# althonos/pyrodigal

Hardware: AMD Instinct MI355X
Metric: Mbp/sec gene-called (meta mode) (higher is better)
Workload: dtype f64; 1 GPU; 100000x20kbp_gc30-70_meta; contigs=100000, bases=2000000000, models=16, contigs_rank0=100000, sub_batch_contigs=6250, contexts_per_gpu=4, genes_all_ranks=2908995, steps_issued=a join of the contexts and a gather per step

## Files before the change

### pyrodigal_amd/csrc/pipeline.hip

```cpp

#include "pga_internal.h"
#include "pipeline.h"
#include <atomic>
#include "dev_common.h"
#include "dpw_core.h"

namespace {

enum { NA = 0, NG = 1, NC = 2, NT = 3, NN = 6 };

__device__ __forceinline__ int find_contig(const ContigDesc* __restrict__ ct, int n, int64_t g) {
    int lo = 0, hi = n - 1;
    while (lo < hi) { int mid = (lo + hi + 1) >> 1; if (ct[mid].base <= g) lo = mid; else hi = mid - 1; }
    return lo;
}

__device__ __forceinline__ int block_contig(const ContigDesc* __restrict__ ct, int n, int64_t block_first, int64_t g, int* s_slot) {
    int c = block_search_le([&](const int k) { return ct[k].base; }, n, block_first, s_slot);
    while (c + 1 < n && ct[c + 1].base <= g) c++;
    return c;
}
__device__ __forceinline__ int block_chain(const ChainDesc* __restrict__ ch, int n, int64_t block_first, int64_t g, int* s_slot) {
    int c = block_search_le([&](const int k) { return ch[k].off; }, n, block_first, s_slot);
    while (c + 1 < n && ch[c + 1].off <= g) c++;
// ... 2184 lines not shown
        if (tid < 256) SM.mot.mk0[tid >> 6][tid & 63] = tm->mot_wt[0][tid >> 6][tid & 63];
#pragma unroll
        for (int e = tid; e < 1024; e += TILE) SM.mot.mk1[e >> 8][e & 255] = tm->mot_wt[1][e >> 8][e & 255];
    }
    if (tid < nj) {
        const SsMmChain C = mm[T.j0 + tid];
        s_item0[tid] = C.item0; s_n[tid] = C.n; s_rdelta[tid] = C.rdelta; s_lf[tid] = C.len_first; s_off[tid] = C.off; s_raw[tid] = C.raw;
    }
    __syncthreads();
    mark(0);
    const int item = T.item0 + tid;
    int lo = 0, hi = nj - 1;
    while (lo < hi) { const int mid = (lo + hi + 1) >> 1; if (s_item0[mid] <= item) lo = mid; else hi = mid - 1; }
    if (item < s_item0[lo] + s_n[lo]) {
    const ulonglong2* const rp = (const ulonglong2*)&rec[item + s_rdelta[lo]];
    const ulonglong2 ra = rp[0], rb = rp[1];
    const int64_t raw = s_raw[lo], g0 = s_off[lo];
    const uint32_t len_first = s_lf[lo];
    const unsigned long long ucodes = ra.x, w1 = ra.y, w2 = rb.x, w3 = rb.y;
    const int i = (int)(unsigned)w3;
    const double cs_raw = ca.cscore_raw[raw + i];
    const int64_t g = g0 + i;
    const int L = (int)(len_first & 0x7fffffffu);
    const bool first = (len_first >> 31) != 0;
    const unsigned long long zm = w1 & ((1ull << 42) - 1ull);
    const int nups = (int)((w1 >> 42) & 63u), start = (int)((w1 >> 48) & 63u), type = (int)((w1 >> 54) & 3u);
    const int strand = ((w1 >> 56) & 1u) ? -1 : 1;
    const bool e0 = (w1 >> 57) & 1u, conv = (w1 >> 58) & 1u, ups_near_edge = (w1 >> 59) & 1u, ups_first = (w1 >> 60) & 1u, ups_later = (w1 >> 61) & 1u;
    const unsigned isA = (unsigned)(w2 & 0xfffffu) << 1, isG = (unsigned)((w2 >> 20) & 0xfffffu) << 1;
    const int stop3 = (int)(w2 >> 40);
    const long orf = (long)(w3 >> 32);
    const bool is_meta = sp.is_meta != 0;
    const double st_wt = SM.st_wt;
    const bool stop_missing = !codon_is_stop(stop3 & 0xff, (stop3 >> 8) & 0xff, (stop3 >> 16) & 0xff, SM.tt);
    const bool edge_in = e0 || (conv && !first);
    mark(1);
    int rbs0 = 0, rbs1 = 0, m_ndx = 0, m_len = 0, m_sp = 0, m_si = 0;
    double m_score = 0.0;
    const bool search_sd = !edge_in && SM.uses_sd, search_mot = !edge_in && !SM.uses_sd;
    auto midx = [&](const int k, const int t2) { return (int)((zm >> (2 * (21 - (18 + k - t2)))) & ((1ull << (2 * (k + 3))) - 1ull)); };
    auto msi = [](const int t2) { return t2 <= 2 ? 3 : (t2 <= 4 ? 2 : (t2 >= 11 ? 1 : 0)); };
    auto upstream = [&]() {
        double v = 0.0;
        unsigned lo32 = (unsigned)ucodes, hi32 = (unsigned)(ucodes >> 32);
        if (nups == 32) {
#pragma unroll
            for (int q = 0; q < 16; q++) { v += SM.ups[q][(lo32 >> (2 * q)) & 3u]; if ((q & 7) == 7) __builtin_amdgcn_sched_barrier(0); }
#pragma unroll
            for (int q = 0; q < 16; q++) { v += SM.ups[16 + q][(hi32 >> (2 * q)) & 3u]; if ((q & 7) == 7) __builtin_amdgcn_sched_barrier(0); }
        } else {
            for (int q = 0; q < nups; q++) v += SM.ups[q][(int)(ucodes >> (2 * q)) & 3];
        }
        return v;
    };
    double u = 0.0;
    if (search_sd) {
        unsigned pats[3] = {0u, 0u, 0u};
#pragma unroll
        for (int q = 0; q < 15; q++) {
            const unsigned a6 = (isA >> (15 - q)) & 63u, g6 = (isG >> (15 - q)) & 63u;
            const unsigned pat = ((a6 >> 5) & 1u) | (((g6 >> 4) & 1u) << 1) | (((g6 >> 3) & 1u) << 2) | (((a6 >> 2) & 1u) << 3) |
                                 (((g6 >> 1) & 1u) << 4) | ((g6 & 1u) << 5);
            pats[q / 5] |= pat << (6 * (q % 5));
        }
#pragma unroll
        for (int q = 0; q < 15; q++) {
            if (start - 20 + q < 0 && strand == 1) continue;
            const unsigned pat = (pats[q / 5] >> (6 * (q % 5))) & 63u;
            const unsigned he = SM.lut[(q << 6) | pat], hm = SM.lut[((15 + q) << 6) | pat];
            if (he > 1u) { const int a = sd_pick(he, SM.rbs_wt); if (a > rbs0) rbs0 = a; }
            if (hm > 1u) { const int b = sd_pick(hm, SM.rbs_wt); if (b > rbs1) rbs1 = b; }
        }
    } else if (search_mot) {
        double bsc = -100.0; int bsp = 0, bsi = 0, blen = 0, bndx = 0;
#pragma unroll 1
        for (int k = 3; k >= 0; k--) {
            const int stride = k == 0 ? 64 : (k == 1 ? 256 : 4096);
            const double* __restrict__ gt = &tm->mot_wt[k][0][0];
            const double* lt = k == 1 ? &SM.mot.mk1[0][0] : &SM.mot.mk0[0][0];
            double scv[13];
            if (k >= 2) {
#pragma unroll
                for (int t2 = 0; t2 < 13; t2++) scv[t2] = 18 + k - t2 > start ? -1000.0 : gt[msi(t2) * stride + midx(k, t2)];
            } else {
#pragma unroll
                for (int t2 = 0; t2 < 13; t2++) scv[t2] = 18 + k - t2 > start ? -1000.0 : lt[msi(t2) * stride + midx(k, t2)];
            }
#pragma unroll
            for (int t2 = 0; t2 < 13; t2++)
                if (scv[t2] > bsc) { bsc = scv[t2]; bsi = msi(t2); bsp = 15 - t2; blen = k + 3; bndx = midx(k, t2); }
        }
        if (bsc == -4.0 || bsc < SM.no_mot + 0.69) { m_score = SM.no_mot; }
        else { m_ndx = bndx; m_len = blen; m_si = bsi; m_sp = bsp & 15; m_score = bsc; }
    }
    if (!edge_in) u = upstream();
    mark(2);
    double edge_gene = 0;
    if (edge_in) edge_gene += 1;
    if (stop_missing) edge_gene += 1;

    double tscore, uscore, rscore, sscore, cscore = cs_raw;
    if (edge_in) {
        tscore = 0.74 * st_wt / edge_gene; uscore = 0.0; rscore = 0.0;
    } else {
        tscore = SM.type_wt[type] * st_wt;
        const double r1 = SM.rbs_wt[rbs0], r2 = SM.rbs_wt[rbs1];
        const double sd = fmax(r1, r2) * st_wt;
        if (SM.uses_sd) rscore = sd;
        else { rscore = st_wt * m_score; if (rscore < sd && SM.no_mot > -0.5) rscore = sd; }
        uscore = u;
        if (ups_near_edge || (first ? ups_first : ups_later)) uscore += -1.00 * st_wt;
    }
    bool edge_now = edge_in;
    if (conv && !edge_in) {
        edge_gene += 1; edge_now = true; tscore = 0.0;
        uscore = 0.74 * st_wt / edge_gene; rscore = 0.0;
    }
    if (!edge_now && edge_gene == 1) uscore -= 0.5 * 0.74 * st_wt;
    if (edge_gene == 0 && orf < 250) {
        const double negf = 250.0 / (float)orf, posf = (float)orf / 250.0;
        rscore *= rscore < 0 ? negf : posf;
        uscore *= uscore < 0 ? negf : posf;
        tscore *= tscore < 0 ? negf : posf;
    }
    if (is_meta && L < 3000 && edge_gene == 0 && (cscore < 5.0 || orf < 120))
        cscore -= 7.5 * fmax(0.0, (3000.0 - L) / 2700.0);
    sscore = tscore + rscore + uscore;
    if (cscore < 0.0) {
        if (edge_gene > 0 && !edge_now) {
            if (!is_meta || L > 1500) sscore -= st_wt; else sscore -= 10.31 - 0.004 * L;
        } else if (is_meta && L < 3000 && edge_now) {
            const double mml = sqrt((double)L) * 5.0;
            if (orf >= mml) { if (cscore >= 0) cscore = -1.0; sscore = 0.0; uscore = 0.0; }
        } else sscore -= 0.5;
    } else if (is_meta && cscore < 5.0 && orf < 120 && sscore < 0.0) sscore -= st_wt;
    mark(3);
    ca.cscore[g] = cscore; ca.sscore[g] = sscore; ca.rscore[g] = rscore; ca.uscore[g] = uscore; ca.tscore[g] = tscore;
    ca.mot_score[g] = m_score; ca.mot_ndx[g] = m_ndx;
    ca.mot_len[g] = (uint8_t)m_len; ca.mot_spacer[g] = (uint8_t)m_sp; ca.mot_spacendx[g] = (uint8_t)m_si;
    ca.rbs[2 * g] = (uint8_t)rbs0; ca.rbs[2 * g + 1] = (uint8_t)rbs1;
    ca.edge[g] = (uint8_t)edge_now;
    if (sp.cs_out != nullptr) sp.cs_out[g] = cscore + sscore;
    mark(4);
    }
}

struct OvlChain {
    const int32_t* __restrict__ ndx; const int32_t* __restrict__ stv; const uint8_t* __restrict__ typ; const int8_t* __restrict__ str;
    const double* __restrict__ cs; const double* __restrict__ ss; const double* __restrict__ rs; const double* __restrict__ us;
    int n;
    const double* __restrict__ css = nullptr;
};
constexpr int OV_SPEC = 16;
__device__ __forceinline__ unsigned overlap_neighbours(const int32_t* __restrict__ ndx, const int32_t* __restrict__ stv, const uint8_t* __restrict__ typ,
                                                       const int8_t* __restrict__ str, const int n, const int i, const int maxov) {
    const int my = ndx[i];
    const bool fwd = str[i] == 1;
    bool ended = false;
    unsigned elig = 0;
    constexpr int OV_NEAR = 10;
#pragma unroll
    for (int k = 0; k < OV_SPEC; k++) {
        if (k == OV_NEAR && ended) break;
        const int j = fwd ? i + 3 - k : i - 3 + k;
        const int jj = min(max(j, 0), n - 1);
        const int nd = ndx[jj], sv = stv[jj], ty = typ[jj], sd = str[jj];
        bool stop_here, ok;
        if (fwd) {
            stop_here = j < 0 || (j < n && nd <= my + 2 && nd + maxov < my);
            ok = j >= 0 && j < n && nd <= my + 2 && sd == 1 && ty != PGA_T_STOP && sv > my;
        } else {
            stop_here = j >= n || (j >= 0 && nd >= my - 2 && nd - maxov > my);
            ok = j >= 0 && j < n && nd >= my - 2 && sd == -1 && ty != PGA_T_STOP && sv < my;
        }
        ended = ended || stop_here;
        if (ok && !ended) {
            elig |= 1u << k;
            if (k < 15 && (fwd ? (my + 2 == nd || my == nd + 1) : (nd + 2 == my || nd == my + 1))) elig |= 0x10000u << k;
        }
    }
    return elig | (ended ? 0x80000000u : 0u);
}

__device__ __forceinline__ void overlapping_starts_of(const OvlChain& C, const int i, const ModelConst* __restrict__ mc, const int maxov,
                                                      int& sp0, int& sp1, int& sp2, const unsigned neighbours) {
    const int32_t* __restrict__ ndx = C.ndx; const int32_t* __restrict__ stv = C.stv;
    const uint8_t* __restrict__ typ = C.typ; const int8_t* __restrict__ str = C.str;
    const double* __restrict__ cs = C.cs; const double* __restrict__ ss = C.ss; const double* __restrict__ rs = C.rs; const double* __restrict__ us = C.us;
    const int n = C.n;
    const int my = ndx[i];
    double best = -100;
    const bool fwd = str[i] == 1;
    const double rs_i = 0.0, us_i = 0.0;
    unsigned elig = neighbours & 0xffffu;
    int js = fwd ? i + 3 - OV_SPEC : i - 3 + OV_SPEC;
    bool more = !(neighbours >> 31);
    for (;;) {
        int j = -1;
        if (elig) {
            const int k = __builtin_ctz(elig);
            elig &= elig - 1u;
            j = fwd ? i + 3 - k : i - 3 + k;
        } else {
            while (more) {
                if (fwd ? js < 0 : js >= n) { more = false; break; }
                const int jq = js;
                js += fwd ? -1 : 1;
                if (jq < 0 || jq >= n) continue;
                const int nq = ndx[jq];
                if (fwd ? nq > my + 2 : nq < my - 2) continue;
                if (fwd ? nq + maxov < my : nq - maxov > my) { more = false; break; }
                if (str[jq] != (fwd ? 1 : -1) || typ[jq] == PGA_T_STOP) continue;
                if (fwd ? stv[jq] <= my : stv[jq] >= my) continue;
                j = jq;
                break;
            }
            if (j < 0) break;
        }
        const int nj = ndx[j];
        const double csj = C.css != nullptr ? C.css[j] : cs[j] + ss[j];
        const bool adj = fwd ? (my + 2 == nj || my == nj + 1) : (nj + 2 == my || nj == my + 1);
        const double rj = adj ? rs[j] : 0.0, uj = adj ? us[j] : 0.0;
        const double v = fwd ? csj + igm_same_dev(my, 1, rs_i, us_i, nj, rj, uj, mc->st_wt, mc->igm)
                             : csj + igm_same_dev(nj, -1, rj, uj, my, rs_i, us_i, mc->st_wt, mc->igm);
        if (v > best) { const int f = nj % 3; if (f == 0) sp0 = j; else if (f == 1) sp1 = j; else sp2 = j; best = v; }
    }
}

__global__ void __launch_bounds__(256)
k_ovl_topo(GroupArrays ga, const int32_t* __restrict__ cbase, const int32_t* __restrict__ sbase, int n_contigs, int n_stops, int maxov) {
    __shared__ int s_c0;
    const int blk0 = blockIdx.x * blockDim.x, s = blk0 + threadIdx.x;
    int c = block_search_le([&](const int k) { return sbase[k]; }, n_contigs, blk0, &s_c0);
    if (s >= n_stops) return;
    while (c + 1 < n_contigs && sbase[c + 1] <= s) c++;
    const int b0 = cbase[c], n = cbase[c + 1] - b0;
    const int i = ga.stop_list[s] - b0;
    if (ga.srank != nullptr) ga.srank[b0 + i] = s - sbase[c];
    ga.ovl_topo[s] = ga.edge0[b0 + i] == 1 ? 0x80000000u
                                           : overlap_neighbours(ga.ndx + b0, ga.stop_val + b0, ga.type + b0, ga.strand + b0, n, i, maxov);
}

__global__ void __launch_bounds__(256)
k_overlapping_starts(const ChainDesc* __restrict__ chains, int n_chains, int64_t node_begin, int64_t total,
                     GroupArrays ga, const ModelConst* __restrict__ mcs, ChainArrays ca, int maxov) {
    __shared__ int s_c0;
    const int64_t blk0 = node_begin + (int64_t)blockIdx.x * blockDim.x;
    const int64_t g = blk0 + threadIdx.x;
    const bool in_range = g < node_begin + total;
    const int c = block_chain(chains, n_chains, blk0, in_range ? g : blk0, &s_c0);
    if (!in_range) return;
    const ChainDesc ch = chains[c];
    const int i = (int)(g - ch.off);
    const int64_t tb = ch.topo_off;
    int sp0 = -1, sp1 = -1, sp2 = -1;
    if (ga.type[tb + i] == PGA_T_STOP && ga.edge0[tb + i] != 1) {
        const OvlChain C{ga.ndx + tb, ga.stop_val + tb, ga.type + tb, ga.strand + tb, ca.cscore + ch.off, ca.sscore + ch.off, ca.rscore + ch.off,
                         ca.uscore + ch.off, ch.n};
        overlapping_starts_of(C, i, &mcs[ch.model], maxov, sp0, sp1, sp2, overlap_neighbours(C.ndx, C.stv, C.typ, C.str, C.n, i, maxov));
    }
    ca.star_ptr[3 * g] = sp0; ca.star_ptr[3 * g + 1] = sp1; ca.star_ptr[3 * g + 2] = sp2;
}

constexpr int OV_AHEAD = 4;
struct OvlKept { double v[3]; int nd[3], sv[3], q2[3]; };
__device__ __forceinline__ void overlapping_starts_ahead(const OvlChain& C, const int i, const int my, const bool fwd, const ModelConst* __restrict__ mc,
                                                         const int maxov, int (&sp)[3], OvlKept& K, const unsigned neighbours,
                                                         const int32_t* __restrict__ q2 ) {
    const int32_t* __restrict__ ndx = C.ndx; const int32_t* __restrict__ stv = C.stv;
    const uint8_t* __restrict__ typ = C.typ; const int8_t* __restrict__ str = C.str;
    const double* __restrict__ cs = C.cs; const double* __restrict__ ss = C.ss; const double* __restrict__ rs = C.rs; const double* __restrict__ us = C.us;
    const int n = C.n;
    const bool rext = !fwd && q2 != nullptr;
    double best = -100;
    unsigned elig = neighbours & 0xffffu;
    const unsigned adjb = (neighbours >> 16) & 0x7fffu;
    int jn[OV_AHEAD], nq[OV_AHEAD], svq[OV_AHEAD], q2q[OV_AHEAD]; double cq[OV_AHEAD], rq[OV_AHEAD], uq[OV_AHEAD]; bool aq[OV_AHEAD];
#pragma unroll
    for (int q = 0; q < OV_AHEAD; q++) {
        jn[q] = -1; aq[q] = false;
        if (elig) { const int k = __builtin_ctz(elig); elig &= elig - 1u; jn[q] = fwd ? i + 3 - k : i - 3 + k; aq[q] = (adjb >> k) & 1u; }
    }
#pragma unroll
    for (int q = 0; q < OV_AHEAD; q++) {
        const int jj = jn[q] >= 0 ? jn[q] : i;
        nq[q] = ndx[jj]; cq[q] = C.css != nullptr ? C.css[jj] : cs[jj] + ss[jj];
        rq[q] = aq[q] ? rs[jj] : 0.0; uq[q] = aq[q] ? us[jj] : 0.0;
        svq[q] = rext ? stv[jj] : 0; q2q[q] = rext ? q2[jj] : 0;
    }
    auto price = [&](const int j, const int nj, const double csj, const double rj0, const double uj0, const int svj, const int q2j) {
        const bool adj = fwd ? (my + 2 == nj || my == nj + 1) : (nj + 2 == my || nj == my + 1);
        const double rj = adj ? rj0 : 0.0, uj = adj ? uj0 : 0.0;
        const double v = fwd ? csj + igm_same_dev(my, 1, 0.0, 0.0, nj, rj, uj, mc->st_wt, mc->igm)
                             : csj + igm_same_dev(nj, -1, rj, uj, my, 0.0, 0.0, mc->st_wt, mc->igm);
        if (v > best) {
            const int f = nj % 3; best = v;
            if (f == 0) { sp[0] = j; K.v[0] = v; K.nd[0] = nj; K.sv[0] = svj; K.q2[0] = q2j; }
            else if (f == 1) { sp[1] = j; K.v[1] = v; K.nd[1] = nj; K.sv[1] = svj; K.q2[1] = q2j; }
            else { sp[2] = j; K.v[2] = v; K.nd[2] = nj; K.sv[2] = svj; K.q2[2] = q2j; }
        }
    };
#pragma unroll
    for (int q = 0; q < OV_AHEAD; q++) if (jn[q] >= 0) price(jn[q], nq[q], cq[q], rq[q], uq[q], svq[q], q2q[q]);
    bool more = !(neighbours >> 31);
    if (!elig && !more) return;
    int js = fwd ? i + 3 - OV_SPEC : i - 3 + OV_SPEC;
    for (;;) {
        int j = -1;
        if (elig) {
            const int k = __builtin_ctz(elig);
            elig &= elig - 1u;
            j = fwd ? i + 3 - k : i - 3 + k;
        } else {
            while (more) {
                if (fwd ? js < 0 : js >= n) { more = false; break; }
                const int jq = js;
                js += fwd ? -1 : 1;
                if (jq < 0 || jq >= n) continue;
                const int nqq = ndx[jq];
                if (fwd ? nqq > my + 2 : nqq < my - 2) continue;
                if (fwd ? nqq + maxov < my : nqq - maxov > my) { more = false; break; }
                if (str[jq] != (fwd ? 1 : -1) || typ[jq] == PGA_T_STOP) continue;
                if (fwd ? stv[jq] <= my : stv[jq] >= my) continue;
                j = jq;
                break;
            }
            if (j < 0) break;
        }
        price(j, ndx[j], C.css != nullptr ? C.css[j] : cs[j] + ss[j], rs[j], us[j], rext ? stv[j] : 0, rext ? q2[j] : 0);
    }
}

__global__ void __launch_bounds__(256)
k_ovl_stops(const ChainDesc* __restrict__ chains, int n_chains, int64_t soff_begin, int64_t n_pairs, GroupArrays ga,
            const int32_t* __restrict__ cbase, const int32_t* __restrict__ sbase, const ModelConst* __restrict__ mcs, ChainArrays ca, int maxov,
            const int32_t* __restrict__ topo_q2, DpwExt* __restrict__ ext, const double* __restrict__ css ,
            const int32_t* __restrict__ blk_chain ) {
    __shared__ int s_c0;
    const int64_t blk0 = soff_begin + (int64_t)blockIdx.x * blockDim.x;
    const int64_t p = blk0 + threadIdx.x;
    int c;
    if (blk_chain != nullptr) c = blk_chain[blockIdx.x];
    else c = block_search_le([&](const int k) { return chains[k].soff; }, n_chains, blk0, &s_c0);
    if (p >= soff_begin + n_pairs) return;
    {
        const int64_t s1 = chains[min(c + 1, n_chains - 1)].soff, s2 = chains[min(c + 2, n_chains - 1)].soff, s3 = chains[min(c + 3, n_chains - 1)].soff;
        const int c_in = c;
        c += (c_in + 1 < n_chains && s1 <= p) + (c_in + 2 < n_chains && s2 <= p) + (c_in + 3 < n_chains && s3 <= p);
    }
    while (c + 1 < n_chains && chains[c + 1].soff <= p) c++;
    const ChainDesc ch = chains[c];
    const int64_t tb = ch.topo_off;
    const int sb = sbase[ch.contig], cb = cbase[ch.contig];
    const int sidx = sb + (int)(p - ch.soff);
    const int i = ga.stop_list[sidx] - cb;
    const unsigned neighbours = ga.ovl_topo[sidx];
    const int64_t g = ch.off + i;
    const ModelConst* __restrict__ mc = &mcs[ch.model];
    const int edge0 = ga.edge0[tb + i], my = ga.ndx[tb + i], my_str = ga.strand[tb + i];
    const bool rev = my_str != 1;
    int sp[3] = {-1, -1, -1};
    OvlKept K{{0.0, 0.0, 0.0}, {0, 0, 0}, {0, 0, 0}, {0, 0, 0}};
    const OvlChain C{ga.ndx + tb, ga.stop_val + tb, ga.type + tb, ga.strand + tb, ca.cscore + ch.off, ca.sscore + ch.off, ca.rscore + ch.off,
                     ca.uscore + ch.off, ch.n, css != nullptr ? css + ch.off : nullptr};
    overlapping_starts_ahead(C, i, my, !rev, mc, maxov, sp, K, edge0 != 1 ? neighbours : 0x80000000u, ext != nullptr ? topo_q2 + tb : nullptr);
    ca.star_ptr[3 * g] = sp[0]; ca.star_ptr[3 * g + 1] = sp[1]; ca.star_ptr[3 * g + 2] = sp[2];
    if (ext != nullptr) {
        DpwExt e;
        e.vm = 0;
#pragma unroll
        for (int k = 0; k < 3; k++) {
            e.x[k] = 0.0; e.dlo[k] = INT_MAX; e.dhi[k] = INT_MIN; e.cq[k] = DPW_NONE;
            if (sp[k] < 0) continue;
            e.vm |= 1 << k;
            e.x[k] = K.v[k];
            if (rev && e.x[k] > 0.0) {
                const int n3n = K.nd[k], n3s = K.sv[k];
                int hi = n3s + DPW_MAX_OPP_OVLP - 5;
                const int h2 = (n3n + n3s - 6) >> 1;
                if (h2 < hi) hi = h2;
                if (my - 4 < hi) hi = my - 4;
                e.dlo[k] = n3s - 5; e.dhi[k] = hi;
            }
            if (rev) e.cq[k] = K.q2[k];
        }
        ext[p] = e;
    }
}

}

static inline unsigned nblocks(int64_t n, int t) { return (unsigned)((n + t - 1) / t); }

int64_t pga_gc_blocks(int64_t total) { return (total + 1 + 4095) / 4096; }

void pga_launch_digitize(const char* d_seq, uint8_t* d_dig, int64_t total, const ContigDesc* d_ct, int n_contigs,
                         int32_t* d_gc, int32_t* d_unk, hipStream_t st) {
    if (total <= 0) return;
    hipLaunchKernelGGL(k_digitize, dim3(nblocks(total, DG_BLOCK)), dim3(256), 0, st, d_seq, d_dig, total, d_ct, n_contigs, d_gc, d_unk);
}

struct RunOfUnknown {
    static __device__ __forceinline__ bool is(const uint8_t b) { return b == NN; }
    static __device__ __forceinline__ bool all8(const uint64_t w) { return w == 0x0606060606060606ull; }
};
struct RunOfLowerCase {
    static __device__ __forceinline__ bool is(const uint8_t b) { return (unsigned)(b - 'a') < 26u; }
    static __device__ __forceinline__ bool all8(const uint64_t w) {
        const uint64_t H = 0x8080808080808080ull;
        if (w & H) return false;
        return ((w + 0x1f1f1f1f1f1f1f1full) & H) == H
            && ((w + 0x0505050505050505ull) & H) == 0;
    }
};

template <class Run, class Emit>
__device__ __forceinline__ void find_runs(const uint8_t* __restrict__ src, const ContigDesc* __restrict__ ct, const TileDesc* __restrict__ tiles,
                                          const int n_tiles, const int n_contigs, const int min_mask, Emit emit) {
    if ((int)blockIdx.x >= n_tiles) {
        const int c = ((int)blockIdx.x - n_tiles) * blockDim.x + threadIdx.x;
        if (c >= n_contigs) return;
        const ContigDesc cd = ct[c];
        if (cd.len < 1 || cd.len > 2) return;
        const uint8_t* __restrict__ d = src + cd.base;
        for (int i = 0; i < cd.len; i++) {
            if (!Run::is(d[i]) || (i > 0 && Run::is(d[i - 1]))) continue;
            int e = i + 1;
            while (e < cd.len && Run::is(d[e])) e++;
            if (e - i >= min_mask || e == cd.len) emit(c, i, e);
        }
        return;
    }
    const TileDesc td = tiles[blockIdx.x];
    const ContigDesc cd = ct[td.contig];
    const int L = cd.len;
    const uint8_t* __restrict__ d = src + cd.base;
    const int i0 = td.start + threadIdx.x * EX_PER_THREAD;
    for (int q = 0; q < EX_PER_THREAD; q++) {
        const int i = i0 + q;
        if (i >= L || !Run::is(d[i]) || (i > 0 && Run::is(d[i - 1]))) continue;
        int e = i + 1;
        while (e + 8 <= L) {
            uint64_t w; memcpy(&w, d + e, 8);
            if (!Run::all8(w)) break;
            e += 8;
        }
        while (e < L && Run::is(d[e])) e++;
        if (e - i >= min_mask || e == L) emit(td.contig, i, e);
    }
}

__global__ void __launch_bounds__(256)
k_find_masks(const uint8_t* __restrict__ dig, const ContigDesc* __restrict__ ct, const TileDesc* __restrict__ tiles, int n_tiles, int n_contigs,
             int min_mask, MaskRun* __restrict__ runs, int32_t* __restrict__ count, int cap) {
    find_runs<RunOfUnknown>(dig, ct, tiles, n_tiles, n_contigs, min_mask, [&](const int c, const int b, const int e) {
        const int k = atomicAdd(count, 1);
        if (k < cap) runs[k] = MaskRun{c, b, e, 0};
    });
}

void pga_launch_find_masks(const uint8_t* d_dig, const ContigDesc* d_ct, int n_contigs, const TileDesc* d_tiles, int n_tiles, int min_mask,
                           MaskRun* d_runs, int32_t* d_count, int cap, hipStream_t st) {
    (void)hipMemsetAsync(d_count, 0, sizeof(int32_t), st);
    hipLaunchKernelGGL(k_find_masks, dim3(n_tiles + (n_contigs + 255) / 256), dim3(256), 0, st, d_dig, d_ct, d_tiles, n_tiles, n_contigs, min_mask,
                       d_runs, d_count, cap);
}

constexpr int MK_WAVE_BITS = 64 * 32;

__device__ __forceinline__ void paint_words(uint32_t* __restrict__ bits, const int64_t g0, const int64_t g1 , const int first, const int step) {
    const int64_t w0 = g0 >> 5, w1 = (g1 - 1) >> 5;
    for (int64_t w = w0 + first; w <= w1; w += step) {
        uint32_t m = 0xffffffffu;
        if (w == w0) m &= 0xffffffffu << (int)(g0 & 31);
        if (w == w1) m &= 0xffffffffu >> (31 - (int)((g1 - 1) & 31));
        atomicOr(bits + w, m);
    }
}

template <class Run>
__global__ void __launch_bounds__(256)
k_mask_paint_runs(const uint8_t* __restrict__ src, const ContigDesc* __restrict__ ct, const TileDesc* __restrict__ tiles, int n_tiles, int n_contigs,
                  int min_mask, uint32_t* __restrict__ bits) {
    find_runs<Run>(src, ct, tiles, n_tiles, n_contigs, min_mask, [&](const int c, const int b, const int e) {
        const int64_t base = ct[c].base;
        paint_words(bits, base + b, base + e, 0, 1);
    });
}

__global__ void __launch_bounds__(256)
k_mask_paint_regions(const MaskRun* __restrict__ regions, int n_regions, const ContigDesc* __restrict__ ct, int n_contigs,
                     uint32_t* __restrict__ bits, uint32_t* __restrict__ cbits) {
    const int region_blocks = (n_regions + 3) / 4;
    if ((int)blockIdx.x >= region_blocks) {
        const int c = ((int)blockIdx.x - region_blocks) * 256 + threadIdx.x;
        if (c < n_contigs) { const int64_t g = ct[c].base; atomicOr(cbits + (g >> 5), 1u << (int)(g & 31)); }
        return;
    }
    const int k = (int)blockIdx.x * 4 + (threadIdx.x >> 6);
    if (k >= n_regions) return;
    const MaskRun r = regions[k];
    const ContigDesc cd = ct[r.contig];
    const int b = max(r.begin, 0), e = min(r.end, cd.len);
    if (b < e) paint_words(bits, cd.base + b, cd.base + e, threadIdx.x & 63, 64);
}

__device__ __forceinline__ void mask_edges(const uint32_t* __restrict__ bits, const uint32_t* __restrict__ cbits, const int64_t w, const int64_t nw,
                                           uint32_t& S, uint32_t& E) {
    S = 0; E = 0;
    if (w >= nw) return;
    const uint32_t b = bits[w];
    if (!b) return;
    const uint32_t before = w > 0 ? bits[w - 1] >> 31 : 0u, after = w + 1 < nw ? bits[w + 1] & 1u : 0u;
    const uint32_t c = cbits[w], c_after = w + 1 < nw ? cbits[w + 1] & 1u : 0u;
    S = b & (~((b << 1) | before) | c);
    E = b & (~((b >> 1) | (after << 31)) | ((c >> 1) | (c_after << 31)));
}

__global__ void __launch_bounds__(256)
k_mask_count(const uint32_t* __restrict__ bits, const uint32_t* __restrict__ cbits, int64_t nw, int32_t* __restrict__ cnt_s, int32_t* __restrict__ cnt_e) {
    const int64_t w = (int64_t)blockIdx.x * 256 + threadIdx.x;
    uint32_t S, E;
    mask_edges(bits, cbits, w, nw, S, E);
    int ns = __popc(S), ne = __popc(E);
#pragma unroll
    for (int m = 32; m >= 1; m >>= 1) { ns += __shfl_xor(ns, m, 64); ne += __shfl_xor(ne, m, 64); }
    if ((threadIdx.x & 63) == 0 && w < nw) { cnt_s[w >> 6] = ns; cnt_e[w >> 6] = ne; }
}

__global__ void __launch_bounds__(256)
k_mask_place(const uint32_t* __restrict__ bits, const uint32_t* __restrict__ cbits, int64_t nw, int word_blocks, const int32_t* __restrict__ off_s,
             const int32_t* __restrict__ off_e, const ContigDesc* __restrict__ ct, int n_contigs, int32_t* __restrict__ moff, int2* __restrict__ iv, int cap) {
    if ((int)blockIdx.x >= word_blocks) {
        const int c = ((int)blockIdx.x - word_blocks) * 256 + threadIdx.x;
        if (c > n_contigs) return;
        const int64_t g = ct[c].base, wg = g >> 5;
        int n = off_s[g / MK_WAVE_BITS];
        uint32_t S, E;
        for (int64_t w = (g / MK_WAVE_BITS) * 64; w < wg; w++) { mask_edges(bits, cbits, w, nw, S, E); n += __popc(S); }
// ... 165 lines not shown
    const int L = ok ? pool[2 * (size_t)s + 1] : 0;
    const double gc = L > 0 ? (double)pool[2 * (size_t)s] / (double)L : 0.0;
    const double low = fmin(0.65, 0.88495 * gc - 0.0102337), high = fmax(0.35, 0.86596 * gc + 0.1131991);
    unsigned need = 0;
    for (int m = 0; m < n_models; m++) if (!(model_gc[m] < low || model_gc[m] > high)) need |= 1u << model_group[m];
    for (int g = 0; g < n_groups; g++) enabled[(size_t)g * n_contigs + i] = (need >> g) & 1;
}
void pga_launch_group_enable_sets(const ContigDesc* d_ct, int n_contigs, const int32_t* d_gc_count, const int32_t* d_set_of, int32_t* d_pool,
                                  const double* d_model_gc, const int32_t* d_model_group, int n_models, int n_groups, uint8_t* d_enabled,
                                  hipStream_t st) {
    if (n_contigs <= 0) return;
    (void)hipMemsetAsync(d_pool, 0, sizeof(int32_t) * 2 * (size_t)n_contigs, st);
    hipLaunchKernelGGL(k_set_pool, dim3(nblocks(n_contigs, 256)), dim3(256), 0, st, d_ct, n_contigs, d_gc_count, d_set_of, d_pool);
    hipLaunchKernelGGL(k_group_enable_sets, dim3(nblocks(n_contigs, 256)), dim3(256), 0, st, n_contigs, d_set_of, d_pool, d_model_gc, d_model_group,
                       n_models, n_groups, d_enabled);
}



void pga_launch_orf_gc(const ContigDesc* d_ct, int n_contigs, const uint8_t* d_dig, const int32_t* d_p16, const GroupArrays& ga,
                       int n_nodes_total, const int32_t* d_node_contig_base, hipStream_t st) {
    if (n_nodes_total <= 0) return;
    hipLaunchKernelGGL(k_orf_gc, dim3(nblocks(n_nodes_total, 256)), dim3(256), 0, st, d_ct, n_contigs, d_dig, d_p16, ga,
                       n_nodes_total, d_node_contig_base);
}

void pga_launch_sd_lut(unsigned* d_lut, hipStream_t st) {
    hipLaunchKernelGGL(k_sd_lut, dim3((PGA_SD_LUT + 255) / 256), dim3(256), 0, st, d_lut);
}

int pga_mm_tile_items() {
    const char* e = getenv("PGA_SS_MM_TILE");
    const int v = e ? atoi(e) : 0;
    return v == 256 || v == 512 || v == 1024 ? v : SS_TILE_DEFAULT;
}
int32_t pga_mm_tiles(const ChainDesc* h_chains, int n_chains, const int32_t* h_cbase, const int32_t* h_sbase, int n_models, std::vector<int64_t>& items) {
    const int tile = pga_mm_tile_items();
    items.assign((size_t)n_models, 0);
    for (int k = 0; k < n_chains; k++) {
        const int c = h_chains[k].contig;
        items[(size_t)h_chains[k].model] += (h_cbase[c + 1] - h_cbase[c]) - (h_sbase[c + 1] - h_sbase[c]);
    }
    int64_t tiles = 0;
    for (int m = 0; m < n_models; m++) tiles += (items[(size_t)m] + tile - 1) / tile;
    return (int32_t)tiles;
}
size_t pga_mm_scratch_bytes(int n_models, int n_chains) {
    return sizeof(unsigned long long) * SS_CNT_STRIDE * (size_t)n_models + sizeof(int32_t) * (((size_t)3 * n_models + 1) & ~(size_t)1) + sizeof(int2) * (size_t)n_chains + 64;
}

void pga_launch_score(const ChainDesc* d_chains, int n_chains, int64_t node_begin, int64_t total, const uint8_t* d_dig,
                      const ContigDesc* d_ct, const GroupArrays& ga, const pga_training* d_models,
                      const ModelScoreConst* d_msc, const ModelConst* d_mc, const ChainArrays& ca, ScoreParams sp,
                      const ChainDesc* d_all_chains, const int2* d_contig_chains, const int32_t* d_node_contig_base, int n_contigs,
                      int group_nodes, const unsigned* d_sd_lut, hipStream_t st, int reuse_raw_cscore, const double* d_gil, int il_stride,
                      const int32_t* d_rank, const void* d_cs_tasks, int n_cs_tasks, const void* d_cs_entries, const StopLaunch* stops) {
    if (total <= 0 || n_chains <= 0) return;
    const dim3 grid(nblocks(total, 256)), blk(256);
    if (group_nodes > 0 && !reuse_raw_cscore && n_cs_tasks > 0) {
        static std::atomic<bool> attr_set[64];
        static std::atomic<unsigned long long*> prof_of[64];
        int dev = 0;
        (void)hipGetDevice(&dev);
        dev &= 63;
        const size_t lds = sizeof(double) * 4096 * 4;
        int cs_wave = CS_WAVE;
        if (const char* e = getenv("PGA_CS_WAVE")) cs_wave = atoi(e) >= 64 ? atoi(e) : CS_WAVE;
        if (!attr_set[dev].load()) {
            hipFuncSetAttribute((const void*)k_coding_score_quads, hipFuncAttributeMaxDynamicSharedMemorySize, (int)lds);
            attr_set[dev].store(true);
        }
        const bool profiling = getenv("PGA_CS_PROFILE") != nullptr;
        unsigned long long* d_prof = prof_of[dev].load();
        if (profiling) {
            if (!d_prof) { (void)hipMalloc((void**)&d_prof, 16 * sizeof(unsigned long long)); prof_of[dev].store(d_prof); }
            (void)hipMemsetAsync(d_prof, 0, 16 * sizeof(unsigned long long), st);
        }
        hipLaunchKernelGGL(k_coding_score_quads, dim3((unsigned)n_cs_tasks), dim3(CS_TASK_THREADS), lds, st, (const CsTask*)d_cs_tasks,
                           (const CsEntry*)d_cs_entries, d_all_chains, d_contig_chains, d_node_contig_base, d_dig, d_ct, ga, d_models, d_msc, ca,
                           d_gil, il_stride, d_rank, cs_wave, profiling ? d_prof : nullptr, (getenv("PGA_CS_QCLASSES") && atoi(getenv("PGA_CS_QCLASSES")) == 4) ? 4 : 3);
        if (profiling) {
            unsigned long long h[16];
            (void)hipStreamSynchronize(st);
            (void)hipMemcpy(h, d_prof, sizeof h, hipMemcpyDeviceToHost);
            fprintf(stderr, "[pga cs-profile] %d tasks (%llu workgroups, %llu batches of 64): wave-cycles  stage %.3g  list %.3g  one-wave ORFs %.3g  "
                            "four-to-a-wave %.3g  64-to-a-wave %.3g (lookup %.3g  first loads %.3g  walk %.3g  penalties %.3g)  end barrier %.3g\n",
                    n_cs_tasks, h[7], h[8], (double)h[0], (double)h[1], (double)h[2], (double)h[3], (double)h[4], (double)h[9], (double)h[10], (double)h[11],
                    (double)h[12], (double)h[5]);
        }
        reuse_raw_cscore = 1;
    }
    if (group_nodes > 0 && !reuse_raw_cscore)
        hipLaunchKernelGGL(k_coding_score, dim3(nblocks(group_nodes, 256)), blk, 0, st, d_all_chains, d_contig_chains, d_node_contig_base,
                           n_contigs, 0, group_nodes, d_dig, d_ct, ga, d_models, d_msc, ca, d_gil, il_stride, d_rank);
    if (group_nodes > 0) {
        if (const char* e = getenv("PGA_SS_MODELS_PER_PASS")) { const int v = atoi(e); if (v >= 1 && v <= 512) sp.models_per_pass = v; }
        static std::atomic<unsigned long long*> ss_prof_of[64];
        const bool ss_profiling = getenv("PGA_SS_PROFILE") != nullptr;
        if (ss_profiling) {
            int dev = 0; (void)hipGetDevice(&dev); dev &= 63;
            unsigned long long* d_prof = ss_prof_of[dev].load();
            if (!d_prof) { (void)hipMalloc((void**)&d_prof, 16 * sizeof(unsigned long long)); ss_prof_of[dev].store(d_prof); }
            (void)hipMemsetAsync(d_prof, 0, 16 * sizeof(unsigned long long), st);
            sp.prof = d_prof;
        }
        const bool listed = stops != nullptr && stops->starts_only && ga.start_list != nullptr;
        const int n_items = listed ? stops->n_starts : group_nodes;
        const bool mm = listed && n_items > 0 && stops->mm_tiles > 0 && stops->mm_rec != nullptr && !(getenv("PGA_SS_MM") && atoi(getenv("PGA_SS_MM")) == 0);
        if (mm) {
            const int nm = sp.n_models;
            unsigned long long* const d_cnt = (unsigned long long*)stops->mm_scratch;
            int32_t* const d_base = (int32_t*)(d_cnt + (size_t)SS_CNT_STRIDE * nm);
            int2* const d_slot = (int2*)(d_base + (((size_t)3 * nm + 1) & ~(size_t)1));
            (void)hipMemsetAsync(d_cnt, 0, sizeof(unsigned long long) * SS_CNT_STRIDE * (size_t)nm, st);
            hipLaunchKernelGGL(k_start_prologue, dim3(nblocks(n_items, 256)), blk, 0, st, d_contig_chains, d_node_contig_base, n_contigs, d_dig, d_ct, ga, sp,
                               (const int32_t*)ga.start_list, n_items, (SsStartRec*)stops->mm_rec);
            hipLaunchKernelGGL(k_mm_count, dim3(nblocks(n_chains, 256)), blk, 0, st, d_chains, n_chains, d_node_contig_base, stops->sbase, nm, d_cnt, d_slot);
            const int tile = pga_mm_tile_items();
            hipLaunchKernelGGL(k_mm_scan, dim3(1), blk, 0, st, (const unsigned long long*)d_cnt, nm, tile, d_base);
            hipLaunchKernelGGL(k_mm_place, dim3(nblocks(n_chains, 256)), blk, 0, st, d_chains, n_chains, d_node_contig_base, stops->sbase, d_ct,
                               (const unsigned long long*)d_cnt, (const int2*)d_slot, (const int32_t*)d_base, nm, tile, d_models, (SsMmChain*)stops->mm_chain, (SsMmTile*)stops->mm_tile);
            const SsMmTile* const d_tl = (const SsMmTile*)stops->mm_tile; const SsMmChain* const d_mc = (const SsMmChain*)stops->mm_chain;
            const SsStartRec* const d_rec = (const SsStartRec*)stops->mm_rec;
            const dim3 grid_mm((unsigned)stops->mm_tiles);
            if (tile == 1024) hipLaunchKernelGGL(k_score_starts_mm<1024>, grid_mm, dim3(1024), 0, st, d_tl, d_mc, d_rec, d_models, ca, sp, d_sd_lut);
            else if (tile == 512) hipLaunchKernelGGL(k_score_starts_mm<512>, grid_mm, dim3(512), 0, st, d_tl, d_mc, d_rec, d_models, ca, sp, d_sd_lut);
            else hipLaunchKernelGGL(k_score_starts_mm<256>, grid_mm, blk, 0, st, d_tl, d_mc, d_rec, d_models, ca, sp, d_sd_lut);
            if (stops->n_stops > 0)
                hipLaunchKernelGGL(k_clear_stops, dim3(nblocks(stops->n_stops, 256)), blk, 0, st, d_all_chains, d_contig_chains, d_node_contig_base, ga, ca, sp,
                                   stops->n_stops);
        } else if (n_items > 0)
            hipLaunchKernelGGL(k_score_starts<4>, dim3(nblocks(n_items, 256)), blk, 0, st, d_all_chains, d_contig_chains, d_node_contig_base, n_contigs,
                               group_nodes, d_dig, d_ct, ga, d_models, ca, sp, d_sd_lut, listed ? (const int32_t*)ga.start_list : (const int32_t*)nullptr, n_items);
        if (ss_profiling && mm) {
            unsigned long long h[16];
            (void)hipStreamSynchronize(st);
            (void)hipMemcpy(h, sp.prof, sizeof h, hipMemcpyDeviceToHost);
            fprintf(stderr, "[pga ss-profile] model-major, %d starts, %d tiles: wave-cycles  stage %.3g  chain + record %.3g  upstream + RBS / motif search %.3g  "
                            "scores %.3g  stores %.3g\n", n_items, stops->mm_tiles, (double)h[0], (double)h[1], (double)h[2], (double)h[3], (double)h[4]);
        } else if (ss_profiling) {
            unsigned long long h[16];
            (void)hipStreamSynchronize(st);
            (void)hipMemcpy(h, sp.prof, sizeof h, hipMemcpyDeviceToHost);
            fprintf(stderr, "[pga ss-profile] %d nodes: wave-cycles  locate %.3g  node + upstream window %.3g  barrier + edge scan %.3g | per model: next model %.3g  "
                            "chain %.3g  upstream + RBS / motif search %.3g  scores %.3g  finish + stores (slot 8) %.3g  stage %.3g  barrier %.3g (slot 7 unused %.3g)\n",
                    group_nodes, (double)h[0], (double)h[1], (double)h[2], (double)h[3], (double)h[4], (double)h[5], (double)h[6], (double)h[8],
                    (double)h[9], (double)h[10], (double)h[7]);
        }
    }
    if (stops != nullptr) {
        if (stops->fill_star_ptr) (void)hipMemsetAsync(ca.star_ptr + 3 * node_begin, 0xff, sizeof(int32_t) * 3 * (size_t)total, st);
        if (stops->n_pairs > 0 && stops->n_stops > 0)
            hipLaunchKernelGGL(k_ovl_topo, dim3(nblocks(stops->n_stops, 256)), blk, 0, st, ga, d_node_contig_base, stops->sbase, n_contigs, stops->n_stops,
                               sp.max_overlap);
        if (stops->n_pairs > 0)
            hipLaunchKernelGGL(k_ovl_stops, dim3(nblocks(stops->n_pairs, 256)), blk, 0, st, d_chains, n_chains, stops->soff_begin, stops->n_pairs, ga,
                               d_node_contig_base, stops->sbase, d_mc, ca, sp.max_overlap, stops->topo_q2, (DpwExt*)stops->ext,
                               stops->ext != nullptr ? (const double*)sp.cs_out : nullptr, getenv("PGA_OVL_SEARCH") ? nullptr : stops->blk_chain);
    } else hipLaunchKernelGGL(k_overlapping_starts, grid, blk, 0, st, d_chains, n_chains, node_begin, total, ga, d_mc, ca, sp.max_overlap);
}
```

Baseline: 21250 Mbp/s.

## Stage overlap-topology node spans in LDS and coalesce extras record stores

k_ovl_topo now cooperatively copies the block's contiguous node span (ndx, stop value, type, edge, strand) into shared memory and runs the neighbour scan from LDS when the window fits, falling back to global memory otherwise. k_ovl_stops transposes each thread's 64-byte DpwExt record through padded shared memory so the block writes ext with coalesced 16-byte stores. This targets scattered global reads and strided wide stores. The cost is extra LDS use, which may lower occupancy, plus a block barrier; out-of-range threads now stay alive so they can reach that barrier.

```diff
diff --git a/pyrodigal_amd/csrc/pipeline.hip b/pyrodigal_amd/csrc/pipeline.hip
--- a/pyrodigal_amd/csrc/pipeline.hip
+++ b/pyrodigal_amd/csrc/pipeline.hip
@@ -2360,8 +2360,42 @@
     const double* __restrict__ css = nullptr;
 };
 constexpr int OV_SPEC = 16;
-__device__ __forceinline__ unsigned overlap_neighbours(const int32_t* __restrict__ ndx, const int32_t* __restrict__ stv, const uint8_t* __restrict__ typ,
-                                                       const int8_t* __restrict__ str, const int n, const int i, const int maxov) {
+
+constexpr int OVL_WINDOW = OV_SPEC - 4;
+constexpr int OVL_MARGIN = OV_SPEC;
+constexpr int OVL_ITER = 6;
+constexpr int OVL_CAP_TOPO = 1536;
+static_assert(OVL_CAP_TOPO <= 256 * OVL_ITER, "a span is copied in OVL_ITER rounds of 256 elements");
+template <class T> using lds_ptr = const __attribute__((address_space(3))) T*;
+template <class T>
+struct Staged {
+    lds_ptr<T> lds; int lo;
+    __device__ __forceinline__ T operator[](const int j) const { return lds[j - lo]; }
+};
+template <class Load, class Store>
+__device__ __forceinline__ void stage_span(const int n, const Load load, const Store store) {
+    decltype(load(0, 0)) r[OVL_ITER];
+#pragma unroll
+    for (int q = 0; q < OVL_ITER; q++) if (256 * q < n) r[q] = load((int)threadIdx.x + 256 * q, 256 * q);
+#pragma unroll
+    for (int q = 0; q < OVL_ITER; q++) if (256 * q < n) store((int)threadIdx.x + 256 * q, r[q]);
+}
+__device__ __forceinline__ bool window_staged(const int i, const int n, const int lo, const int len) {
+    return max(i - OVL_WINDOW, 0) >= lo && min(i + OVL_WINDOW, n - 1) < lo + len;
+}
+__device__ __forceinline__ void span_of(const int64_t first, const int64_t last, const int64_t lo_bound, const int64_t hi_bound, const int cap,
+                                        int64_t& begin, int& n) {
+    begin = max(first - OVL_MARGIN, lo_bound);
+    n = (int)min(min(last + OVL_MARGIN + 1, hi_bound) - begin, (int64_t)cap);
+    if (n < 0) n = 0;
+}
+static int ovl_cap(const int kernel_cap) {
+    const char* e = getenv("PGA_OVL_CAP");
+    return (e ? std::max(0, std::min(kernel_cap, atoi(e))) : kernel_cap) & ~3;
+}
+
+template <class Ndx, class Stv, class Typ, class Str>
+__device__ __forceinline__ unsigned overlap_neighbours(const Ndx ndx, const Stv stv, const Typ typ, const Str str, const int n, const int i, const int maxov) {
     const int my = ndx[i];
     const bool fwd = str[i] == 1;
     bool ended = false;
@@ -2436,17 +2470,36 @@
 }
 
 __global__ void __launch_bounds__(256)
-k_ovl_topo(GroupArrays ga, const int32_t* __restrict__ cbase, const int32_t* __restrict__ sbase, int n_contigs, int n_stops, int maxov) {
+k_ovl_topo(GroupArrays ga, const int32_t* __restrict__ cbase, const int32_t* __restrict__ sbase, int n_contigs, int n_stops, int maxov,
+           const int cap ) {
     __shared__ int s_c0;
+    __shared__ int32_t s_ndx[OVL_CAP_TOPO], s_stv[OVL_CAP_TOPO];
+    __shared__ uint8_t s_typ[OVL_CAP_TOPO], s_e0[OVL_CAP_TOPO];
+    __shared__ int8_t s_str[OVL_CAP_TOPO];
     const int blk0 = blockIdx.x * blockDim.x, s = blk0 + threadIdx.x;
     int c = block_search_le([&](const int k) { return sbase[k]; }, n_contigs, blk0, &s_c0);
+    int64_t t0; int nt;
+    span_of(ga.stop_list[blk0], ga.stop_list[min(blk0 + 255, n_stops - 1)], 0, cbase[n_contigs], cap, t0, nt);
+    struct Node { int32_t ndx, stv; uint8_t typ, e0; int8_t str; };
+    stage_span(nt, [&](const int k, int) { const int64_t t = t0 + (k < nt ? k : 0);
+                                           return Node{ga.ndx[t], ga.stop_val[t], ga.type[t], ga.edge0[t], ga.strand[t]}; },
+               [&](const int k, const Node& v) { if (k < nt) { s_ndx[k] = v.ndx; s_stv[k] = v.stv; s_typ[k] = v.typ; s_e0[k] = v.e0; s_str[k] = v.str; } });
+    __syncthreads();
     if (s >= n_stops) return;
     while (c + 1 < n_contigs && sbase[c + 1] <= s) c++;
     const int b0 = cbase[c], n = cbase[c + 1] - b0;
     const int i = ga.stop_list[s] - b0;
     if (ga.srank != nullptr) ga.srank[b0 + i] = s - sbase[c];
-    ga.ovl_topo[s] = ga.edge0[b0 + i] == 1 ? 0x80000000u
-                                           : overlap_neighbours(ga.ndx + b0, ga.stop_val + b0, ga.type + b0, ga.strand + b0, n, i, maxov);
+    const int lo = (int)t0 - b0;
+    unsigned r;
+    if (window_staged(i, n, lo, nt)) {
+        const Staged<int32_t> ndx{(lds_ptr<int32_t>)s_ndx, lo}, stv{(lds_ptr<int32_t>)s_stv, lo};
+        const Staged<uint8_t> typ{(lds_ptr<uint8_t>)s_typ, lo}, e0{(lds_ptr<uint8_t>)s_e0, lo};
+        const Staged<int8_t> str{(lds_ptr<int8_t>)s_str, lo};
+        r = e0[i] == 1 ? 0x80000000u : overlap_neighbours(ndx, stv, typ, str, n, i, maxov);
+    } else
+        r = ga.edge0[b0 + i] == 1 ? 0x80000000u : overlap_neighbours(ga.ndx + b0, ga.stop_val + b0, ga.type + b0, ga.strand + b0, n, i, maxov);
+    ga.ovl_topo[s] = r;
 }
 
 __global__ void __launch_bounds__(256)
@@ -2539,18 +2592,22 @@
     }
 }
 
+constexpr int OVL_EXT_PITCH = 257, OVL_EXT_SLOTS = 4 * OVL_EXT_PITCH;
+static_assert(sizeof(DpwExt) == 64, "an extras record is four 16-byte pieces");
 __global__ void __launch_bounds__(256)
 k_ovl_stops(const ChainDesc* __restrict__ chains, int n_chains, int64_t soff_begin, int64_t n_pairs, GroupArrays ga,
             const int32_t* __restrict__ cbase, const int32_t* __restrict__ sbase, const ModelConst* __restrict__ mcs, ChainArrays ca, int maxov,
             const int32_t* __restrict__ topo_q2, DpwExt* __restrict__ ext, const double* __restrict__ css ,
             const int32_t* __restrict__ blk_chain ) {
     __shared__ int s_c0;
+    __shared__ uint4 s_ext[OVL_EXT_SLOTS];
+    const int tid = threadIdx.x;
     const int64_t blk0 = soff_begin + (int64_t)blockIdx.x * blockDim.x;
-    const int64_t p = blk0 + threadIdx.x;
+    const bool valid = blk0 + tid < soff_begin + n_pairs;
+    const int64_t p = valid ? blk0 + tid : soff_begin + n_pairs - 1;
     int c;
     if (blk_chain != nullptr) c = blk_chain[blockIdx.x];
     else c = block_search_le([&](const int k) { return chains[k].soff; }, n_chains, blk0, &s_c0);
-    if (p >= soff_begin + n_pairs) return;
     {
         const int64_t s1 = chains[min(c + 1, n_chains - 1)].soff, s2 = chains[min(c + 2, n_chains - 1)].soff, s3 = chains[min(c + 3, n_chains - 1)].soff;
         const int c_in = c;
@@ -2572,7 +2629,7 @@
     const OvlChain C{ga.ndx + tb, ga.stop_val + tb, ga.type + tb, ga.strand + tb, ca.cscore + ch.off, ca.sscore + ch.off, ca.rscore + ch.off,
                      ca.uscore + ch.off, ch.n, css != nullptr ? css + ch.off : nullptr};
     overlapping_starts_ahead(C, i, my, !rev, mc, maxov, sp, K, edge0 != 1 ? neighbours : 0x80000000u, ext != nullptr ? topo_q2 + tb : nullptr);
-    ca.star_ptr[3 * g] = sp[0]; ca.star_ptr[3 * g + 1] = sp[1]; ca.star_ptr[3 * g + 2] = sp[2];
+    if (valid) { ca.star_ptr[3 * g] = sp[0]; ca.star_ptr[3 * g + 1] = sp[1]; ca.star_ptr[3 * g + 2] = sp[2]; }
     if (ext != nullptr) {
         DpwExt e;
         e.vm = 0;
@@ -2592,7 +2649,15 @@
             }
             if (rev) e.cq[k] = K.q2[k];
         }
-        ext[p] = e;
+        uint4 w[4];
+        memcpy(w, &e, sizeof e);
+#pragma unroll
+        for (int q = 0; q < 4; q++) s_ext[q * OVL_EXT_PITCH + tid] = w[q];
+        __syncthreads();
+        const int n_out = 4 * (int)min((int64_t)256, soff_begin + n_pairs - blk0);
+        uint4* const out = (uint4*)(ext + blk0);
+#pragma unroll
+        for (int q = 0; q < 4; q++) { const int o = tid + 256 * q; if (o < n_out) out[o] = s_ext[(o & 3) * OVL_EXT_PITCH + (o >> 2)]; }
     }
 }
 
@@ -3064,7 +3129,7 @@
         if (stops->fill_star_ptr) (void)hipMemsetAsync(ca.star_ptr + 3 * node_begin, 0xff, sizeof(int32_t) * 3 * (size_t)total, st);
         if (stops->n_pairs > 0 && stops->n_stops > 0)
             hipLaunchKernelGGL(k_ovl_topo, dim3(nblocks(stops->n_stops, 256)), blk, 0, st, ga, d_node_contig_base, stops->sbase, n_contigs, stops->n_stops,
-                               sp.max_overlap);
+                               sp.max_overlap, ovl_cap(OVL_CAP_TOPO));
         if (stops->n_pairs > 0)
             hipLaunchKernelGGL(k_ovl_stops, dim3(nblocks(stops->n_pairs, 256)), blk, 0, st, d_chains, n_chains, stops->soff_begin, stops->n_pairs, ga,
                                d_node_contig_base, stops->sbase, d_mc, ca, sp.max_overlap, stops->topo_q2, (DpwExt*)stops->ext,
```

Result: no change. 21210 Mbp/s (-0.2%).
